# nv-tlabs/GEN3C

Measured on NVIDIA H100. Metric: denoise-steps/sec, 7B DiT, 121-frame 720p latent, higher is better.
Workload: dtype bf16

## Files before the change

### gen3c_b200/csrc/attn_wgmma.cu

```cuda
#include <cmath>
#include <cstdlib>

#include "kernels.h"

namespace g3c {

constexpr int ATT_THREADS = 384;
constexpr int ATT_TILE = 128;
constexpr int ATT_HALF_BYTES = 128 * 128;
constexpr int ATT_TILE_BYTES = 2 * ATT_HALF_BYTES;
constexpr int ATT_STAGES = 2;
constexpr int ATT_SMEM = ATT_TILE_BYTES + ATT_STAGES * 2 * ATT_TILE_BYTES + 256 + 1024;

struct AttnParams {
  int Lq, Lk, heads;
  int ldo;
  int vt_chunk_len;
  __nv_bfloat16* O;
  float scale_log2;
  const uint32_t* chunk_flags;
  uint32_t flag_seq;
  int first_chunk;
  unsigned long long peer_timeout_ns;
  unsigned long long* wait_ns;
  unsigned long long* trace;
};

static unsigned long long* g_attn_trace = nullptr;

#define ATT_TR(role, slot)                                                                                  \
  do {                                                                                                      \
    if constexpr (kTrace) {                                                                                 \
      if (blockIdx.x == 0 && blockIdx.y == 0 && j < 64 && (threadIdx.x % 128) == 0)                         \
        p.trace[((role) * 64 + j) * 8 + (slot)] = clock64();                                                \
    }                                                                                                       \
  } while (0)

__device__ __forceinline__ float ex2_approx(float x) {
  float y;
  asm("ex2.approx.ftz.f32 %0, %1;\n" : "=f"(y) : "f"(x));
  return y;
}

template <bool kTrace>
__global__ void __launch_bounds__(ATT_THREADS, 1)
    k_attn_fwd(const __grid_constant__ CUtensorMap tmQ, const __grid_constant__ CUtensorMap tmK,
               const __grid_constant__ CUtensorMap tmV, const AttnParams p) {
  extern __shared__ uint8_t smem_raw[];
  uint8_t* smem = reinterpret_cast<uint8_t*>((reinterpret_cast<uintptr_t>(smem_raw) + 1023) &
                                             ~static_cast<uintptr_t>(1023));
  uint8_t* smem_q = smem;
  uint8_t* smem_k = smem + ATT_TILE_BYTES;
  uint8_t* smem_v = smem_k + ATT_STAGES * ATT_TILE_BYTES;
  uint64_t* bars = reinterpret_cast<uint64_t*>(smem_v + ATT_STAGES * ATT_TILE_BYTES);
  uint64_t* q_full = bars;
  uint64_t* k_full = bars + 1;
  uint64_t* v_full = bars + 1 + ATT_STAGES;
  uint64_t* kv_empty = bars + 1 + 2 * ATT_STAGES;

  const uint32_t wg = threadIdx.x / 128;
  const uint32_t tid = threadIdx.x % 128;
  const int head = blockIdx.y;
  const int q0 = blockIdx.x * ATT_TILE;
  const int n_kv = p.Lk / ATT_TILE;

  if (threadIdx.x == 0) {
    tma_prefetch_desc(&tmQ);
    tma_prefetch_desc(&tmK);
    tma_prefetch_desc(&tmV);
    mbar_init(q_full, 1);
    for (int i = 0; i < ATT_STAGES; ++i) {
      mbar_init(&k_full[i], 1);
      mbar_init(&v_full[i], 1);
      mbar_init(&kv_empty[i], 2);
    }
    fence_barrier_init();
  }
  __syncthreads();

  if (wg == 0) {
    setmaxnreg_dec<24>();
    if (tid == 0) {
      mbar_expect_tx(q_full, ATT_TILE_BYTES);
      for (int h = 0; h < 2; ++h) tma_load_2d(smem_q + h * ATT_HALF_BYTES, &tmQ, q_full, head * 128 + h * 64, q0);
      const int tiles_per_chunk = p.vt_chunk_len / ATT_TILE;
      const int n_chunks = p.Lk / p.vt_chunk_len;
      uint32_t stage = 0, phase = 0;
      for (int j = 0; j < n_kv; ++j) {
        int chunk = p.first_chunk + j / tiles_per_chunk;
        if (chunk >= n_chunks) chunk -= n_chunks;
        const int within = j % tiles_per_chunk;
        if (p.chunk_flags && within == 0 && chunk != p.first_chunk) {
          uint32_t v, spins = 0;
          uint64_t t0 = 0;
          for (;;) {
            asm volatile("ld.acquire.sys.global.u32 %0, [%1];\n" : "=r"(v) : "l"(p.chunk_flags + chunk) : "memory");
            if ((int)(v - p.flag_seq) >= 0) break;
            if (t0 == 0) t0 = global_timer_ns();
            if ((++spins & 0x3FFu) == 0 && global_timer_ns() - t0 > p.peer_timeout_ns) asm volatile("trap;\n");
          }
          if (t0 != 0 && p.wait_ns) atomicAdd(p.wait_ns, (unsigned long long)(global_timer_ns() - t0));
          asm volatile("fence.proxy.async.global;\n" ::: "memory");
        }
        const int kv0 = chunk * p.vt_chunk_len + within * ATT_TILE;
        mbar_wait_ns(&kv_empty[stage], phase ^ 1, p.peer_timeout_ns);
        mbar_expect_tx(&k_full[stage], ATT_TILE_BYTES);
        for (int h = 0; h < 2; ++h)
          tma_load_2d(smem_k + stage * ATT_TILE_BYTES + h * ATT_HALF_BYTES, &tmK, &k_full[stage], head * 128 + h * 64,
                      kv0);
        mbar_expect_tx(&v_full[stage], ATT_TILE_BYTES);
        for (int h = 0; h < 2; ++h)
          tma_load_3d(smem_v + stage * ATT_TILE_BYTES + h * ATT_HALF_BYTES, &tmV, &v_full[stage],
                      within * ATT_TILE + h * 64, head * 128, chunk);
        if (++stage == ATT_STAGES) {
          stage = 0;
          phase ^= 1;
        }
      }
    }
  } else {
    setmaxnreg_inc<240>();
    const uint32_t c = wg - 1;
    const uint32_t warp = tid / 32, lane = tid % 32;
    float o[64];
#pragma unroll
    for (int i = 0; i < 64; ++i) o[i] = 0.f;
    float m_run[2] = {-INFINITY, -INFINITY};
    float l_run[2] = {0.f, 0.f};
    const float sl2 = p.scale_log2;
    const uint64_t dq = make_sdesc_sw128(smem_u32(smem_q + c * 64 * 128));
    mbar_wait_ns(q_full, 0, p.peer_timeout_ns);
    uint32_t stage = 0, phase = 0;
    for (int j = 0; j < n_kv; ++j) {
      ATT_TR(1 + c, 0);
      float s[64];
      mbar_wait_ns(&k_full[stage], phase, p.peer_timeout_ns);
      ATT_TR(1 + c, 1);
      {
        const uint64_t dk = make_sdesc_sw128(smem_u32(smem_k + stage * ATT_TILE_BYTES));
        wgmma_fence();
#pragma unroll
        for (int kk = 0; kk < 8; ++kk) {
          const uint32_t off = (kk >> 2) * ATT_HALF_BYTES + (kk & 3) * 32;
          wgmma_ss_n128(s, sdesc_advance(dq, off), sdesc_advance(dk, off), kk > 0 ? 1u : 0u);
        }
        wgmma_commit();
        wgmma_wait<0>();
        fence_regs(s);
      }
      ATT_TR(1 + c, 2);
      float mx[2] = {-INFINITY, -INFINITY};
#pragma unroll
      for (int i = 0; i < 16; ++i) {
        mx[0] = fmaxf(mx[0], fmaxf(s[4 * i], s[4 * i + 1]));
        mx[1] = fmaxf(mx[1], fmaxf(s[4 * i + 2], s[4 * i + 3]));
      }
      float alpha[2], nm[2];
#pragma unroll
      for (int h = 0; h < 2; ++h) {
        mx[h] = fmaxf(mx[h], __shfl_xor_sync(0xffffffffu, mx[h], 1));
        mx[h] = fmaxf(mx[h], __shfl_xor_sync(0xffffffffu, mx[h], 2));
        nm[h] = fmaxf(m_run[h], mx[h] * sl2);
        alpha[h] = ex2_approx(m_run[h] - nm[h]);
        m_run[h] = nm[h];
        l_run[h] *= alpha[h];
      }
      uint32_t pa[32];
#pragma unroll
      for (int i = 0; i < 16; ++i) {
        const float p0 = ex2_approx(fmaf(s[4 * i], sl2, -nm[0])), p1 = ex2_approx(fmaf(s[4 * i + 1], sl2, -nm[0]));
        const float p2 = ex2_approx(fmaf(s[4 * i + 2], sl2, -nm[1])), p3 = ex2_approx(fmaf(s[4 * i + 3], sl2, -nm[1]));
        l_run[0] += p0 + p1;
        l_run[1] += p2 + p3;
        pa[2 * i] = pack_bf16x2(p0, p1);
        pa[2 * i + 1] = pack_bf16x2(p2, p3);
      }
#pragma unroll
      for (int i = 0; i < 16; ++i) {
        o[4 * i] *= alpha[0];
        o[4 * i + 1] *= alpha[0];
        o[4 * i + 2] *= alpha[1];
        o[4 * i + 3] *= alpha[1];
      }
      ATT_TR(1 + c, 3);
      mbar_wait_ns(&v_full[stage], phase, p.peer_timeout_ns);
      {
        const uint64_t dv = make_sdesc_sw128(smem_u32(smem_v + stage * ATT_TILE_BYTES));
        wgmma_fence();
#pragma unroll
        for (int kk = 0; kk < 8; ++kk) {
          const uint32_t a[4] = {pa[4 * kk], pa[4 * kk + 1], pa[4 * kk + 2], pa[4 * kk + 3]};
          wgmma_rs_n128(o, a, sdesc_advance(dv, (kk >> 2) * ATT_HALF_BYTES + (kk & 3) * 32));
        }
        wgmma_commit();
        wgmma_wait<0>();
        fence_regs(o);
      }
      if (tid == 0) mbar_arrive(&kv_empty[stage]);
      ATT_TR(1 + c, 4);
      if (++stage == ATT_STAGES) {
        stage = 0;
        phase ^= 1;
      }
    }
    float inv[2];
#pragma unroll
    for (int h = 0; h < 2; ++h) {
      float l = l_run[h];
      l += __shfl_xor_sync(0xffffffffu, l, 1);
      l += __shfl_xor_sync(0xffffffffu, l, 2);
      inv[h] = 1.0f / l;
    }
    const int row_a = q0 + (int)(c * 64 + warp * 16 + lane / 4);
#pragma unroll
    for (int h = 0; h < 2; ++h) {
      const int row = row_a + 8 * h;
      if (row >= p.Lq) continue;
      __nv_bfloat16* dst = p.O + (size_t)row * p.ldo + head * 128 + 2 * (lane % 4);
#pragma unroll
      for (int i = 0; i < 16; ++i)
        *reinterpret_cast<uint32_t*>(dst + 8 * i) = pack_bf16x2(o[4 * i + 2 * h] * inv[h], o[4 * i + 2 * h + 1] * inv[h]);
    }
  }
}

int attn_fwd(const void* q, const void* k, const void* vt, void* o, int Lq, int Lk, int heads,
             int ldq, int ldk, int ldo, int vt_chunk_len, float scale, cudaStream_t st, const ChunkGate* gate) {
  G3C_REQUIRE(q && k && vt && o, "attn: null operand");
  G3C_REQUIRE(Lq > 0 && Lk > 0 && heads > 0, "attn: bad sizes");
  G3C_REQUIRE(Lk % ATT_TILE == 0, "attn: Lk=%d must be a multiple of 128", Lk);
  if (vt_chunk_len <= 0) vt_chunk_len = Lk;
  G3C_REQUIRE(Lk % vt_chunk_len == 0 && vt_chunk_len % ATT_TILE == 0,
              "attn: vt_chunk_len=%d must divide Lk=%d and be a multiple of 128", vt_chunk_len, Lk);
  G3C_REQUIRE(ldq % 8 == 0 && ldk % 8 == 0 && ldo % 8 == 0 && ldq >= heads * 128 &&
                  ldk >= heads * 128 && ldo >= heads * 128,
              "attn: leading dimensions must be >= heads*128 and multiples of 8");
  G3C_REQUIRE((reinterpret_cast<uintptr_t>(o) & 15) == 0, "attn: O must be 16-byte aligned");
  CUtensorMap tmQ, tmK, tmV;
  {
    uint64_t dims[2] = {(uint64_t)heads * 128, (uint64_t)Lq}, str[1] = {(uint64_t)ldq * 2};
    uint32_t box[2] = {64, 128};
    int rc = make_tmap_bf16_sw128(&tmQ, q, 2, dims, str, box);
    if (rc) return rc;
  }
  {
    uint64_t dims[2] = {(uint64_t)heads * 128, (uint64_t)Lk}, str[1] = {(uint64_t)ldk * 2};
    uint32_t box[2] = {64, 128};
    int rc = make_tmap_bf16_sw128(&tmK, k, 2, dims, str, box);
    if (rc) return rc;
  }
  {
    const int chunks = Lk / vt_chunk_len;
    uint64_t dims[3] = {(uint64_t)vt_chunk_len, (uint64_t)heads * 128, (uint64_t)chunks};
    uint64_t str[2] = {(uint64_t)vt_chunk_len * 2, (uint64_t)vt_chunk_len * 2 * heads * 128};
    uint32_t box[3] = {64, 128, 1};
    int rc = make_tmap_bf16_sw128(&tmV, vt, 3, dims, str, box);
    if (rc) return rc;
  }
  static bool configured = false;
  if (!configured) {
    G3C_CUDA(cudaFuncSetAttribute(k_attn_fwd<false>, cudaFuncAttributeMaxDynamicSharedMemorySize, ATT_SMEM));
    G3C_CUDA(cudaFuncSetAttribute(k_attn_fwd<true>, cudaFuncAttributeMaxDynamicSharedMemorySize, ATT_SMEM));
    configured = true;
  }
  AttnParams p;
  p.Lq = Lq;
  p.Lk = Lk;
  p.heads = heads;
  p.ldo = ldo;
  p.vt_chunk_len = vt_chunk_len;
  p.O = reinterpret_cast<__nv_bfloat16*>(o);
  p.scale_log2 = scale * 1.4426950408889634f;
  if (fabsf(p.scale_log2 - 1.0f) < 1e-6f) p.scale_log2 = 1.0f;
  p.chunk_flags = gate ? gate->flags : nullptr;
  p.peer_timeout_ns = gate ? peer_timeout_ns() : G3C_MBAR_TIMEOUT_NS;
  p.wait_ns = gate ? gate->wait_ns : nullptr;
  p.flag_seq = gate ? gate->seq : 0;
  p.first_chunk = gate ? gate->first : 0;
  p.trace = g_attn_trace;
  G3C_REQUIRE(p.first_chunk >= 0 && p.first_chunk < Lk / vt_chunk_len, "attn: first chunk %d out of range", p.first_chunk);
  dim3 grid((Lq + ATT_TILE - 1) / ATT_TILE, heads);
  if (g_attn_trace) k_attn_fwd<true><<<grid, ATT_THREADS, ATT_SMEM, st>>>(tmQ, tmK, tmV, p);
  else k_attn_fwd<false><<<grid, ATT_THREADS, ATT_SMEM, st>>>(tmQ, tmK, tmV, p);
  G3C_CUDA(cudaGetLastError());
  return G3C_OK;
}

}

extern "C" int g3c_attn_set_trace(unsigned long long* device_buffer) {
  g3c::g_attn_trace = device_buffer;
  return G3C_OK;
}

extern "C" int g3c_attn_fwd(const void* q, const void* k, const void* vt, void* o, int Lq, int Lk,
                            int heads, int ldq, int ldk, int ldo, int vt_chunk_len, float scale,
                            void* stream) {
  return g3c::attn_fwd(q, k, vt, o, Lq, Lk, heads, ldq, ldk, ldo, vt_chunk_len, scale,
                       (cudaStream_t)stream, nullptr);
}
```

### gen3c_b200/csrc/common.cuh

```cuda
#pragma once
#include <cuda.h>
#include <cuda_bf16.h>
#include <cuda_runtime.h>
#include <stdint.h>
#include <stdio.h>

#include "../../include/gen3c_b200.h"
#include "wgmma_ops.cuh"

namespace g3c {

void set_error(const char* fmt, ...);
int cuda_fail(cudaError_t e, const char* what, const char* file, int line);
#define G3C_CUDA(x)                                                         \
  do {                                                                      \
    cudaError_t _e = (x);                                                   \
    if (_e != cudaSuccess) return ::g3c::cuda_fail(_e, #x, __FILE__, __LINE__); \
  } while (0)
#define G3C_REQUIRE(cond, ...)        \
  do {                                \
    if (!(cond)) {                    \
      ::g3c::set_error(__VA_ARGS__);  \
      return G3C_EINVAL;       \
    }                                 \
  } while (0)

int make_tmap_bf16_sw128(CUtensorMap* out, const void* base, int rank, const uint64_t* dims,
                         const uint64_t* strides_bytes, const uint32_t* box);
int make_tmap_f32_sw128(CUtensorMap* out, const void* base, const uint64_t* dims,
                        const uint64_t* strides_bytes, const uint32_t* box);

int sm_count();

#ifdef __CUDACC__
__device__ __forceinline__ uint32_t smem_u32(const void* p) {
  return static_cast<uint32_t>(__cvta_generic_to_shared(p));
}
__device__ __forceinline__ uint32_t lane_id() { return threadIdx.x & 31; }
__device__ __forceinline__ uint32_t warp_id() { return __shfl_sync(0xffffffffu, threadIdx.x >> 5, 0); }

__device__ __forceinline__ bool elect_one() {
  uint32_t pred = 0;
  asm volatile(
      "{\n\t.reg .pred P;\n\t"
      "elect.sync _|P, 0xffffffff;\n\t"
      "selp.b32 %0, 1, 0, P;\n\t}\n"
      : "=r"(pred));
  return pred != 0;
}

__device__ __forceinline__ void mbar_init(uint64_t* bar, uint32_t count) {
  asm volatile("mbarrier.init.shared::cta.b64 [%0], %1;\n" ::"r"(smem_u32(bar)), "r"(count));
}
__device__ __forceinline__ void fence_barrier_init() {
  asm volatile("fence.mbarrier_init.release.cluster;\n" ::: "memory");
}
__device__ __forceinline__ void fence_proxy_async() {
  asm volatile("fence.proxy.async.shared::cta;\n" ::: "memory");
}
__device__ __forceinline__ void mbar_expect_tx(uint64_t* bar, uint32_t bytes) {
  asm volatile("mbarrier.arrive.expect_tx.shared::cta.b64 _, [%0], %1;\n" ::"r"(smem_u32(bar)),
               "r"(bytes)
               : "memory");
}
__device__ __forceinline__ void mbar_arrive(uint64_t* bar) {
  asm volatile("mbarrier.arrive.shared::cta.b64 _, [%0];\n" ::"r"(smem_u32(bar)) : "memory");
}
#ifndef G3C_MBAR_SUSPEND_NS
#define G3C_MBAR_SUSPEND_NS 0
#endif
__device__ __forceinline__ bool mbar_try_wait(uint64_t* bar, uint32_t parity) {
  uint32_t ok;
#if G3C_MBAR_SUSPEND_NS > 0
  asm volatile(
      "{\n\t.reg .pred P;\n\t"
      "mbarrier.try_wait.parity.shared::cta.b64 P, [%1], %2, %3;\n\t"
      "selp.b32 %0, 1, 0, P;\n\t}\n"
      : "=r"(ok)
      : "r"(smem_u32(bar)), "r"(parity), "r"((uint32_t)G3C_MBAR_SUSPEND_NS)
      : "memory");
#else
  asm volatile(
      "{\n\t.reg .pred P;\n\t"
      "mbarrier.try_wait.parity.shared::cta.b64 P, [%1], %2;\n\t"
      "selp.b32 %0, 1, 0, P;\n\t}\n"
      : "=r"(ok)
      : "r"(smem_u32(bar)), "r"(parity)
      : "memory");
#endif
  return ok != 0;
}
__device__ __forceinline__ bool mbar_test(uint64_t* bar, uint32_t parity) {
  uint32_t ok;
  asm volatile(
      "{\n\t.reg .pred P;\n\t"
      "mbarrier.test_wait.parity.shared::cta.b64 P, [%1], %2;\n\t"
      "selp.b32 %0, 1, 0, P;\n\t}\n"
      : "=r"(ok)
      : "r"(smem_u32(bar)), "r"(parity)
      : "memory");
  return ok != 0;
}
#ifndef G3C_MBAR_TIMEOUT_NS
#define G3C_MBAR_TIMEOUT_NS 4000000000ull
#endif
__device__ __forceinline__ uint64_t global_timer_ns() {
  uint64_t t;
  asm volatile("mov.u64 %0, %%globaltimer;\n" : "=l"(t));
  return t;
}
#ifdef G3C_MBAR_DEBUG
#define G3C_MBAR_TIMEOUT_ACTION(bar, parity)                                                                 \
  do {                                                                                                       \
    printf("g3c: mbarrier timeout block(%d,%d) thread %d bar@%u parity %u\n", blockIdx.x, blockIdx.y,        \
           threadIdx.x, bar, parity);                                                                        \
    __trap();                                                                                                \
  } while (0)
#else
#define G3C_MBAR_TIMEOUT_ACTION(bar, parity) asm volatile("trap;\n")
#endif
__device__ __forceinline__ void mbar_wait(uint64_t* bar, uint32_t parity) {
  if (mbar_try_wait(bar, parity)) return;
  uint32_t spins = 0;
  uint64_t t0 = 0;
  while (!mbar_try_wait(bar, parity)) {
    if ((++spins & 0xFFFu) == 0) {
      uint64_t now = global_timer_ns();
      if (t0 == 0) t0 = now;
      else if (now - t0 > G3C_MBAR_TIMEOUT_NS) G3C_MBAR_TIMEOUT_ACTION(smem_u32(bar), parity);
    }
  }
}

__device__ __forceinline__ void mbar_wait_ns(uint64_t* bar, uint32_t parity, unsigned long long timeout_ns) {
  if (mbar_try_wait(bar, parity)) return;
  uint32_t spins = 0;
  uint64_t t0 = 0;
  while (!mbar_try_wait(bar, parity)) {
    if ((++spins & 0xFFFu) == 0) {
      uint64_t now = global_timer_ns();
      if (t0 == 0) t0 = now;
      else if (now - t0 > timeout_ns) G3C_MBAR_TIMEOUT_ACTION(smem_u32(bar), parity);
    }
  }
}

__device__ __forceinline__ void tma_prefetch_desc(const CUtensorMap* m) {
  asm volatile("prefetch.tensormap [%0];\n" ::"l"(reinterpret_cast<uint64_t>(m)) : "memory");
}
__device__ __forceinline__ void tma_load_2d(void* smem_dst, const CUtensorMap* m, uint64_t* bar,
                                            int c0, int c1) {
  asm volatile(
      "cp.async.bulk.tensor.2d.shared::cluster.global.mbarrier::complete_tx::bytes"
      " [%0], [%1, {%3, %4}], [%2];\n" ::"r"(smem_u32(smem_dst)),
      "l"(reinterpret_cast<uint64_t>(m)), "r"(smem_u32(bar)), "r"(c0), "r"(c1)
      : "memory");
}
__device__ __forceinline__ void tma_load_3d(void* smem_dst, const CUtensorMap* m, uint64_t* bar,
                                            int c0, int c1, int c2) {
  asm volatile(
      "cp.async.bulk.tensor.3d.shared::cluster.global.mbarrier::complete_tx::bytes"
      " [%0], [%1, {%3, %4, %5}], [%2];\n" ::"r"(smem_u32(smem_dst)),
      "l"(reinterpret_cast<uint64_t>(m)), "r"(smem_u32(bar)), "r"(c0), "r"(c1), "r"(c2)
      : "memory");
}

__device__ __forceinline__ void tma_store_2d(const CUtensorMap* m, const void* smem_src, int c0, int c1) {
  asm volatile("cp.async.bulk.tensor.2d.global.shared::cta.bulk_group [%0, {%2, %3}], [%1];\n" ::"l"(
                   reinterpret_cast<uint64_t>(m)),
               "r"(smem_u32(smem_src)), "r"(c0), "r"(c1)
               : "memory");
}
__device__ __forceinline__ void tma_reduce_add_2d(const CUtensorMap* m, const void* smem_src, int c0, int c1) {
  asm volatile("cp.reduce.async.bulk.tensor.2d.global.shared::cta.add.bulk_group [%0, {%2, %3}], [%1];\n" ::"l"(
                   reinterpret_cast<uint64_t>(m)),
               "r"(smem_u32(smem_src)), "r"(c0), "r"(c1)
               : "memory");
}
__device__ __forceinline__ void tma_store_commit() { asm volatile("cp.async.bulk.commit_group;\n" ::: "memory"); }
template <int N>
__device__ __forceinline__ void tma_store_wait_read() {
  asm volatile("cp.async.bulk.wait_group.read %0;\n" ::"n"(N) : "memory");
}
template <int N>
__device__ __forceinline__ void tma_store_wait_all() {
  asm volatile("cp.async.bulk.wait_group %0;\n" ::"n"(N) : "memory");
}

__device__ __forceinline__ void wgmma_fence() { asm volatile("wgmma.fence.sync.aligned;\n" ::: "memory"); }
__device__ __forceinline__ void wgmma_commit() { asm volatile("wgmma.commit_group.sync.aligned;\n" ::: "memory"); }
template <int N>
__device__ __forceinline__ void wgmma_wait() {
  asm volatile("wgmma.wait_group.sync.aligned %0;\n" ::"n"(N) : "memory");
}
template <int N>
__device__ __forceinline__ void fence_regs(float (&r)[N]) {
#pragma unroll
  for (int i = 0; i < N; ++i) asm volatile("" : "+f"(r[i])::"memory");
}

__device__ __forceinline__ uint64_t make_sdesc_sw128(uint32_t smem_addr) {
  uint64_t d = 0;
  d |= static_cast<uint64_t>((smem_addr & 0x3FFFFu) >> 4);
  d |= static_cast<uint64_t>(1) << 16;
  d |= static_cast<uint64_t>(1024u >> 4) << 32;
  d |= static_cast<uint64_t>(1) << 62;
  return d;
}
__device__ __forceinline__ uint64_t sdesc_advance(uint64_t d, uint32_t bytes) {
  return d + static_cast<uint64_t>(bytes >> 4);
}

template <int N>
__device__ __forceinline__ void setmaxnreg_dec() {
  asm volatile("setmaxnreg.dec.sync.aligned.u32 %0;\n" ::"n"(N));
}
template <int N>
__device__ __forceinline__ void setmaxnreg_inc() {
  asm volatile("setmaxnreg.inc.sync.aligned.u32 %0;\n" ::"n"(N));
}

__device__ __forceinline__ uint32_t pack_bf16x2(float lo, float hi) {
  __nv_bfloat162 v = __floats2bfloat162_rn(lo, hi);
  return *reinterpret_cast<uint32_t*>(&v);
}
__device__ __forceinline__ float warp_max(float v) {
#pragma unroll
  for (int o = 16; o > 0; o >>= 1) v = fmaxf(v, __shfl_xor_sync(0xffffffffu, v, o));
  return v;
}
__device__ __forceinline__ float warp_sum(float v) {
#pragma unroll
  for (int o = 16; o > 0; o >>= 1) v += __shfl_xor_sync(0xffffffffu, v, o);
  return v;
}
#endif

}
```

### gen3c_b200/csrc/dit_engine.cu

```cuda
#include <dlfcn.h>

#include <array>
#include <cmath>
#include <cstdlib>
#include <cstring>
#include <string>
#include <unordered_map>
#include <vector>

#include "kernels.h"

namespace g3c {

typedef struct ncclComm* ncclComm_t;
typedef struct { char internal[128]; } ncclUniqueId;
struct NcclApi {
  int (*GetUniqueId)(ncclUniqueId*) = nullptr;
  int (*CommInitRank)(ncclComm_t*, int, ncclUniqueId, int) = nullptr;
  int (*CommDestroy)(ncclComm_t) = nullptr;
  int (*AllGather)(const void*, void*, size_t, int, ncclComm_t, cudaStream_t) = nullptr;
  int (*GroupStart)() = nullptr;
  int (*GroupEnd)() = nullptr;
  const char* (*GetErrorString)(int) = nullptr;
  bool ok = false;
// ... 242 lines not shown
  if (!v) {
    const char* e = getenv("G3C_PEER_TIMEOUT_S");
    double sec = e ? atof(e) : 600.0;
    if (!(sec > 0)) sec = 600.0;
    v = (unsigned long long)(sec * 1e9);
  }
  return v;
}

static int build_tables(g3c_dit* h, cudaStream_t st) {
  if (h->tables_ready) return G3C_OK;
  const g3c_dit_config& c = h->cfg;
  const int dim = 128, dim_h = dim / 6 * 2, dim_w = dim_h, dim_t = dim - 2 * dim_h;
  const int nt = dim_t / 2, nh = dim_h / 2, nw = dim_w / 2;
  std::vector<float> fr(64);
  auto ntk = [](float ratio, int d) { return powf(ratio, (float)d / (float)(d - 2)); };
  const float th_h = 10000.0f * ntk(c.rope_h_ratio, dim_h), th_w = 10000.0f * ntk(c.rope_w_ratio, dim_w),
              th_t = 10000.0f * ntk(c.rope_t_ratio, dim_t);
  for (int j = 0; j < nt; ++j) fr[j] = 1.0f / powf(th_t, (float)(2 * j) / (float)dim_t);
  for (int j = 0; j < nh; ++j) fr[nt + j] = 1.0f / powf(th_h, (float)(2 * j) / (float)dim_h);
  for (int j = 0; j < nw; ++j) fr[nt + nh + j] = 1.0f / powf(th_w, (float)(2 * j) / (float)dim_w);
  G3C_CUDA(cudaMemcpyAsync(h->freqs, fr.data(), 64 * sizeof(float), cudaMemcpyHostToDevice, st));
  G3C_CUDA(cudaStreamSynchronize(st));
  const int t0 = h->cp_rank * h->T;
  const float t_scale = (1.0f / h->fps) * (float)c.base_fps;
  TRY(rope_table(h->freqs, nt, nh, nw, t0, t_scale, h->T, h->Hp, h->Wp, h->rope, st));
  TRY(abs_pos(h->pos_t, h->pos_h, h->pos_w, t0, h->T, h->Hp, h->Wp, c.model_channels, h->pos, st));
  h->tables_ready = true;
  return G3C_OK;
}

static int forward(g3c_dit* h, const void* x_in, const void* cond_mask, const void* cond_pose,
                   const void* padding_mask, float timestep, const void* ctx, void* out,
                   cudaStream_t st) {
  static_assert(sizeof(float) == 4, "");
  G3C_REQUIRE(h && x_in && cond_mask && ctx && out, "dit_forward: null argument");
  G3C_REQUIRE(h->L > 0, "dit_forward: g3c_dit_set_shape was not called");
  TRY(resolve(h, st));
  TRY(build_tables(h, st));
  const g3c_dit_config& c = h->cfg;
  const int D = c.model_channels, R = c.adaln_lora_dim, F = c.ffn_dim, L = h->L, heads = c.num_heads;
  const int Lk_all = L * h->cp_size;
  const float attn_scale = 0.6931471805599453f;
  static int fuse_nr = -1;
  if (fuse_nr < 0) {
    const char* e = getenv("G3C_FUSE_NORM_ROPE");
    fuse_nr = e ? atoi(e) != 0 : 1;
  }
  auto proj_norm_rope = [&](const void* a, const void* w, __nv_bfloat16* out, int M, int Kin,
                            const float* gamma, const float* cs, int& launches) -> int {
    if (fuse_nr) {
      NormRope nr;
      nr.gamma = gamma;
      nr.cs = cs;
      nr.eps = 1e-6f;
      TRY(prof_mark(h, CAT_GEMM, true, st));
      TRY(gemm_bf16(a, w, out, M, D, Kin, Kin, Kin, D, G3C_EPI_BF16, nullptr, 0, st, nullptr, &nr));
      TRY(prof_mark(h, CAT_GEMM, false, st));
      launches += 1;
    } else {
      TRY(prof_mark(h, CAT_GEMM, true, st));
      TRY(gemm_bf16(a, w, out, M, D, Kin, Kin, Kin, D, G3C_EPI_BF16, nullptr, 0, st));
      TRY(prof_mark(h, CAT_GEMM, false, st));
      TRY(prof_mark(h, CAT_ELTWISE, true, st));
      TRY(rmsnorm_rope(out, D, M, heads, gamma, cs, 1e-6f, st));
      TRY(prof_mark(h, CAT_ELTWISE, false, st));
      launches += 2;
    }
    return G3C_OK;
  };
  int n = 0;

  PatchSrc src;
  src.ptr[0] = (const __nv_bfloat16*)x_in;        src.nch[0] = 16;                      src.per_frame[0] = 1;
  src.ptr[1] = (const __nv_bfloat16*)cond_mask;   src.nch[1] = 1;                       src.per_frame[1] = 1;
  src.ptr[2] = (const __nv_bfloat16*)cond_pose;   src.nch[2] = c.in_channels - 17;      src.per_frame[2] = 1;
  src.ptr[3] = (const __nv_bfloat16*)padding_mask; src.nch[3] = c.concat_padding_mask ? 1 : 0; src.per_frame[3] = 0;
  K(CAT_ELTWISE, patchify(src, h->T, h->Hp, h->Wp, h->Kpad, h->tok, st));
  K(CAT_GEMM, gemm_bf16(h->tok, h->w_patch_pad, h->x, L, D, h->Kpad, h->Kpad, h->Kpad, D, G3C_EPI_F32, nullptr, 0, st));

  if (!(h->mods_valid && h->mods_timestep == timestep)) {
    K(CAT_VECTOR, timestep_embed(timestep, D, h->affine_gamma, 1e-6f, h->vec_s, h->vec_emb, st));
    K(CAT_VECTOR, gemv(h->w_t1, h->vec_s, nullptr, h->vec_h1, D, D, 0, 0, st));
    K(CAT_VECTOR, gemv(h->w_t2, h->vec_h1, nullptr, h->vec_lora, 3 * D, D, 1, 0, st));
    for (int i = 0; i < c.num_blocks; ++i)
      for (int j = 0; j < 3; ++j) {
        const SubBlock& s = h->blk[i][j];
        K(CAT_VECTOR, gemv(s.ada1, h->vec_emb, nullptr, h->vec_a, R, D, 1, 0, st));
        K(CAT_VECTOR, gemv(s.ada2, h->vec_a, h->vec_lora, h->mods + (size_t)(i * 3 + j) * 3 * D, 3 * D, R, 0, 0, st));
      }
    K(CAT_VECTOR, gemv(h->f_ada1, h->vec_emb, nullptr, h->vec_a, R, D, 1, 0, st));
    K(CAT_VECTOR, gemv(h->f_ada2, h->vec_a, h->vec_lora, h->modf, 2 * D, R, 0, 0, st));
    h->mods_valid = true;
    h->mods_timestep = timestep;
  }

  __nv_bfloat16* k_loc = h->k_all + (size_t)h->cp_rank * L * D;
  __nv_bfloat16* vt_loc = h->vt_all + (size_t)h->cp_rank * L * D;

  for (int i = 0; i < c.num_blocks; ++i) {
    {
      const SubBlock& s = h->blk[i][0];
      const float* m = h->mods + (size_t)(i * 3 + 0) * 3 * D;
      K(CAT_ELTWISE, ln_modulate(h->x, h->pos, m, m + D, h->xn, L, D, 1e-6f, st));
      if (h->cp_size > 1 && h->cp_p2p) {
        G3C_REQUIRE(h->peers_open, "dit_forward: context-parallel peers not imported (g3c_dit_cp_import)");
        const uint32_t seq = ++h->kv_seq;
        const int set = seq & 1, me = h->cp_rank;
        const size_t slice = (size_t)L * D * 2;
        char* reg = (char*)h->cp_region;
        __nv_bfloat16* kb = (__nv_bfloat16*)(reg + h->off_k[set]);
        __nv_bfloat16* vb = (__nv_bfloat16*)(reg + h->off_vt[set]);
        __nv_bfloat16* kl = kb + (size_t)me * L * D;
        __nv_bfloat16* vl = vb + (size_t)me * L * D;
        PeerDst pk, pv, pf;
        for (int r = 0; r < h->cp_size; ++r) {
          char* pb = (char*)h->peer_base[r];
          pf.ptr[pf.n++] = pb + h->off_flags + (size_t)(set * 8 + me) * 4;
          if (r == me) continue;
          pk.ptr[pk.n++] = pb + h->off_k[set] + (size_t)me * slice;
          pv.ptr[pv.n++] = pb + h->off_vt[set] + (size_t)me * slice;
        }
        if (h->cp_push_sm) {
          K(CAT_GEMM, gemm_bf16(h->xn, s.wk, kl, L, D, D, D, D, D, G3C_EPI_BF16, nullptr, 0, st));
          K(CAT_COMM, rmsnorm_rope(kl, D, L, heads, s.gk, h->rope, 1e-6f, st, &pk));
          K(CAT_COMM, gemm_bf16(s.wv, h->xn, vl, D, L, D, D, D, L, G3C_EPI_BF16, nullptr, 0, st, &pv));
          k_cp_signal<<<1, 32, 0, st>>>(pf, seq);
          G3C_CUDA(cudaGetLastError());
          ++n;
        } else {
          TRY(proj_norm_rope(h->xn, s.wk, kl, L, D, s.gk, h->rope, n));
          K(CAT_GEMM, gemm_bf16(s.wv, h->xn, vl, D, L, D, D, D, L, G3C_EPI_BF16, nullptr, 0, st));
          G3C_CUDA(cudaEventRecord(h->ev_kv, st));
          G3C_CUDA(cudaStreamWaitEvent(h->comm_stream, h->ev_kv, 0));
          uint32_t* slot = h->seq_ring + (seq % g3c_dit::kSeqRing);
          *slot = seq;
          for (int i2 = 1; i2 < h->cp_size; ++i2) {
            const int r = (me - i2 + h->cp_size) % h->cp_size;
            char* pb = (char*)h->peer_base[r];
            G3C_CUDA(cudaMemcpyAsync(pb + h->off_k[set] + (size_t)me * slice, kl, slice, cudaMemcpyDeviceToDevice,
                                     h->comm_stream));
            G3C_CUDA(cudaMemcpyAsync(pb + h->off_vt[set] + (size_t)me * slice, vl, slice, cudaMemcpyDeviceToDevice,
                                     h->comm_stream));
            G3C_CUDA(cudaMemcpyAsync(pb + h->off_flags + (size_t)(set * 8 + me) * 4, slot, 4, cudaMemcpyHostToDevice,
                                     h->comm_stream));
          }
        }
        TRY(proj_norm_rope(h->xn, s.wq, h->q, L, D, s.gq, h->rope, n));
        ChunkGate gate;
        gate.flags = (const uint32_t*)(reg + h->off_flags) + set * 8;
        gate.seq = seq;
        gate.first = me;
        gate.wait_ns = h->prof ? h->wait_ns : nullptr;
        h->wait_cta_launches = (double)((L + 255) / 256) * heads;
        K(CAT_ATTN_SELF, attn_fwd(h->q, kb, vb, h->att, L, Lk_all, heads, D, D, D, L, attn_scale, st, &gate));
      } else {
        TRY(proj_norm_rope(h->xn, s.wk, k_loc, L, D, s.gk, h->rope, n));
        K(CAT_GEMM, gemm_bf16(s.wv, h->xn, vt_loc, D, L, D, D, D, L, G3C_EPI_BF16, nullptr, 0, st));
        if (h->cp_size > 1) {
          G3C_CUDA(cudaEventRecord(h->ev_kv, st));
          G3C_CUDA(cudaStreamWaitEvent(h->comm_stream, h->ev_kv, 0));
          G3C_NCCL(nccl().GroupStart());
          G3C_NCCL(nccl().AllGather(k_loc, h->k_all, (size_t)L * D, kNcclBfloat16, h->comm, h->comm_stream));
          G3C_NCCL(nccl().AllGather(vt_loc, h->vt_all, (size_t)L * D, kNcclBfloat16, h->comm, h->comm_stream));
          G3C_NCCL(nccl().GroupEnd());
          G3C_CUDA(cudaEventRecord(h->ev_gathered, h->comm_stream));
          n += 2;
        }
        TRY(proj_norm_rope(h->xn, s.wq, h->q, L, D, s.gq, h->rope, n));
        if (h->cp_size > 1) G3C_CUDA(cudaStreamWaitEvent(st, h->ev_gathered, 0));
        K(CAT_ATTN_SELF, attn_fwd(h->q, h->k_all, h->vt_all, h->att, L, Lk_all, heads, D, D, D, L, attn_scale, st));
      }
      K(CAT_GEMM, gemm_bf16(h->att, s.wo, h->x, L, D, D, D, D, D, G3C_EPI_GATED_RESIDUAL_F32, m + 2 * D, 0, st));
    }
    {
      const SubBlock& s = h->blk[i][1];
      const float* m = h->mods + (size_t)(i * 3 + 1) * 3 * D;
      const int C = c.context_dim, M = h->ctx_len;
      K(CAT_ELTWISE, ln_modulate(h->x, nullptr, m, m + D, h->xn, L, D, 1e-6f, st));
      TRY(proj_norm_rope(ctx, s.wk, h->kc, M, C, s.gk, nullptr, n));
      K(CAT_GEMM, gemm_bf16(s.wv, ctx, h->vtc, D, M, C, C, C, M, G3C_EPI_BF16, nullptr, 0, st));
      TRY(proj_norm_rope(h->xn, s.wq, h->q, L, D, s.gq, nullptr, n));
      K(CAT_ATTN_CROSS, attn_fwd(h->q, h->kc, h->vtc, h->att, L, M, heads, D, D, D, M, attn_scale, st));
      K(CAT_GEMM, gemm_bf16(h->att, s.wo, h->x, L, D, D, D, D, D, G3C_EPI_GATED_RESIDUAL_F32, m + 2 * D, 0, st));
    }
    {
      const SubBlock& s = h->blk[i][2];
      const float* m = h->mods + (size_t)(i * 3 + 2) * 3 * D;
      K(CAT_ELTWISE, ln_modulate(h->x, nullptr, m, m + D, h->xn, L, D, 1e-6f, st));
      K(CAT_GEMM, gemm_bf16(h->xn, s.w1, h->hid, L, F, D, D, D, F, G3C_EPI_GELU_BF16, nullptr, 0, st));
      K(CAT_GEMM, gemm_bf16(h->hid, s.w2, h->x, L, D, F, F, F, D, G3C_EPI_GATED_RESIDUAL_F32, m + 2 * D, 0, st));
    }
  }
  const int No = c.out_channels * 4;
  K(CAT_ELTWISE, ln_modulate(h->x, nullptr, h->modf, h->modf + D, h->xn, L, D, 1e-6f, st));
  K(CAT_GEMM, gemm_bf16(h->xn, h->w_final, h->yfin, L, No, D, D, D, No, G3C_EPI_F32, nullptr, 64, st));
  K(CAT_ELTWISE, unpatchify(h->yfin, No, h->T, h->Hp, h->Wp, c.out_channels, (__nv_bfloat16*)out, st));
  h->launches = n;
  return G3C_OK;
}

}

extern "C" {

int g3c_dit_create(const g3c_dit_config* cfg, g3c_dit_t** out) {
  G3C_REQUIRE(cfg && out, "dit_create: null argument");
  G3C_REQUIRE(cfg->model_channels % 128 == 0 && cfg->num_heads * 128 == cfg->model_channels,
              "dit_create: head_dim must be 128 (model_channels=%d heads=%d)", cfg->model_channels,
              cfg->num_heads);
  G3C_REQUIRE(cfg->adaln_lora_dim % 8 == 0 && cfg->context_dim % 8 == 0 && cfg->ffn_dim % 8 == 0,
              "dit_create: adaln_lora_dim/context_dim/ffn_dim must be multiples of 8");
  G3C_REQUIRE(cfg->in_channels >= 17 && cfg->out_channels > 0 && cfg->num_blocks > 0, "dit_create: bad config");
  g3c_dit* h = new g3c_dit();
  h->cfg = *cfg;
  *out = h;
  return G3C_OK;
}

static void free_cp_region(g3c_dit* h) {
  if (h->cp_region || h->cfg_region) cudaDeviceSynchronize();
  if (h->cfg_peer) cudaIpcCloseMemHandle(h->cfg_peer);
  h->cfg_peer = nullptr;
  if (h->cfg_region) cudaFree(h->cfg_region);
  h->cfg_region = nullptr;
  for (int r = 0; r < 8; ++r) {
    if (h->peer_base[r] && h->peer_base[r] != h->cp_region) cudaIpcCloseMemHandle(h->peer_base[r]);
    h->peer_base[r] = nullptr;
  }
  h->peers_open = false;
  if (h->cp_region) cudaFree(h->cp_region);
  h->cp_region = nullptr;
  h->cp_region_bytes = 0;
}

static void free_ws(g3c_dit* h) {
  free_cp_region(h);
  if (h->ws) cudaFree(h->ws);
  h->ws = nullptr;
  h->ws_bytes = 0;
  h->L = 0;
  h->tables_ready = false;
  h->mods_valid = false;
}

int g3c_dit_destroy(g3c_dit_t* h) {
  if (!h) return G3C_OK;
  free_ws(h);
  if (h->w_patch_pad) cudaFree(h->w_patch_pad);
  if (h->gammas) cudaFree(h->gammas);
  if (h->comm && nccl().ok) nccl().CommDestroy(h->comm);
  if (h->comm_stream) cudaStreamDestroy(h->comm_stream);
  if (h->seq_ring) cudaFreeHost(h->seq_ring);
  if (h->wait_ns) cudaFree(h->wait_ns);
  if (h->ev_kv) cudaEventDestroy(h->ev_kv);
  if (h->ev_gathered) cudaEventDestroy(h->ev_gathered);
  for (cudaEvent_t e : h->ev_pool) cudaEventDestroy(e);
  delete h;
  return G3C_OK;
}

int g3c_dit_load(g3c_dit_t* h, const char* name, const void* ptr, const int64_t* shape, int ndim, int dtype) {
  G3C_REQUIRE(h && name && ptr && shape && ndim >= 1 && ndim <= 4, "dit_load: bad arguments");
  WTensor t;
  t.ptr = ptr;
  t.shape.assign(shape, shape + ndim);
  t.dtype = dtype;
  h->w[name] = t;
  h->resolved = false;
  h->tables_ready = false;
  h->mods_valid = false;
  return G3C_OK;
}

int g3c_nccl_unique_id(void* out128) {
  G3C_REQUIRE(out128, "nccl_unique_id: null argument");
  if (!nccl().ok) {
    set_error("libnccl.so.2 could not be loaded");
    return G3C_ENCCL;
  }
  ncclUniqueId id;
  G3C_NCCL(nccl().GetUniqueId(&id));
  memcpy(out128, &id, 128);
  return G3C_OK;
}

int g3c_dit_enable_cp(g3c_dit_t* h, const void* nccl_unique_id, int cp_rank, int cp_size) {
  G3C_REQUIRE(h && cp_size >= 1 && cp_size <= 8 && cp_rank >= 0 && cp_rank < cp_size, "enable_cp: bad arguments");
  if (h->comm && nccl().ok) {
    nccl().CommDestroy(h->comm);
    h->comm = nullptr;
  }
  h->cp_p2p = nccl_unique_id == nullptr;
  {
    const char* e = getenv("G3C_CP_PUSH");
    h->cp_push_sm = e && e[0] == 's';
  }
  if (!h->cp_p2p) {
    if (!nccl().ok) {
      set_error("libnccl.so.2 could not be loaded");
      return G3C_ENCCL;
    }
    ncclUniqueId id;
    memcpy(&id, nccl_unique_id, 128);
    G3C_NCCL(nccl().CommInitRank(&h->comm, cp_size, id, cp_rank));
  }
  if (!h->comm_stream) {
// ... 278 lines not shown
```

### gen3c_b200/csrc/kernels.h

```cpp
#pragma once
#include "common.cuh"

namespace g3c {

struct PeerDst {
  int n = 0;
  void* ptr[8] = {nullptr, nullptr, nullptr, nullptr, nullptr, nullptr, nullptr, nullptr};
};

struct NormRope {
  const float* gamma = nullptr;
  const float* cs = nullptr;
  float eps = 1e-6f;
};

int gemm_bf16(const void* A, const void* B, void* D, int M, int N, int K, int lda, int ldb, int ldd,
              int epilogue, const float* gate, int block_n, cudaStream_t st, const PeerDst* peers = nullptr,
              const NormRope* norm_rope = nullptr);
struct ChunkGate {
  const uint32_t* flags = nullptr;
  uint32_t seq = 0;
  int first = 0;
  unsigned long long* wait_ns = nullptr;
};
unsigned long long peer_timeout_ns();
int attn_fwd(const void* q, const void* k, const void* vt, void* o, int Lq, int Lk, int heads,
             int ldq, int ldk, int ldo, int vt_chunk_len, float scale, cudaStream_t st,
             const ChunkGate* gate = nullptr);

struct PatchSrc {
  const __nv_bfloat16* ptr[4];
  int nch[4];
  int per_frame[4];
};

int ln_modulate(float* x, const __nv_bfloat16* pos, const float* shift, const float* scale,
                __nv_bfloat16* y, int L, int D, float eps, cudaStream_t st);
int rmsnorm_rope(__nv_bfloat16* qk, int ld, int L, int heads, const float* gamma, const float* cs,
                 float eps, cudaStream_t st, const PeerDst* peers = nullptr);
int gemv(const __nv_bfloat16* W, const float* x, const float* add, float* y, int N, int K, int pre,
         int round_out, cudaStream_t st);
int patchify(const PatchSrc& src, int T, int Hp, int Wp, int Kpad, __nv_bfloat16* out, cudaStream_t st);
int unpatchify(const float* y, int ldy, int T, int Hp, int Wp, int C, __nv_bfloat16* out, cudaStream_t st);
int timestep_embed(float t, int D, const __nv_bfloat16* gamma, float eps, float* s, float* emb,
                   cudaStream_t st);
int abs_pos(const __nv_bfloat16* pt, const __nv_bfloat16* ph, const __nv_bfloat16* pw, int t0, int T,
            int Hp, int Wp, int D, __nv_bfloat16* out, cudaStream_t st);
int rope_table(const float* freqs, int nt, int nh, int nw, int t0, float t_scale, int T, int Hp, int Wp,
               float* cs, cudaStream_t st);
int bf16_to_f32(const __nv_bfloat16* in, float* out, size_t n, cudaStream_t st, float scale = 1.0f);
int sampler_pre(const __nv_bfloat16* xt, const __nv_bfloat16* gt, const float* noise, const float* ind_t,
                int C, int T, size_t plane, float sigma, float sigma_aug, float sd,
                __nv_bfloat16* xtilde, __nv_bfloat16* xin, cudaStream_t st);
int sampler_post(const __nv_bfloat16* xtilde, const __nv_bfloat16* oc, const __nv_bfloat16* ou,
                 const __nv_bfloat16* gt, const float* ind_t, int C, int T, size_t plane, float guidance,
                 float sigma, float sigma_next, float sigma_aug, float sd, __nv_bfloat16* xnext,
                 __nv_bfloat16* net_out, cudaStream_t st);

}
```

Measured before the change: 0.09124.

## Software-pipeline attention: overlap next QK^T with softmax and PV, ping-pong warpgroups

Restructures the consumer loop of the wgmma attention kernel so the QK^T for tile j is issued together with the PV product for tile j-1, letting the softmax run while tensor-core work is in flight. It adds turn barriers that alternate wgmma issue between the two consumer warpgroups, and splits the K and V empty barriers so K slots free earlier. Prologue and epilogue handle the first S and the last PV. It also adds an exit-on-timeout wait and a done barrier for the producer. The cost is more live registers (s, pa and o held at once) and extra barrier traffic.

```diff
diff --git a/gen3c_b200/csrc/attn_wgmma.cu b/gen3c_b200/csrc/attn_wgmma.cu
--- a/gen3c_b200/csrc/attn_wgmma.cu
+++ b/gen3c_b200/csrc/attn_wgmma.cu
@@ -6,11 +6,13 @@
 namespace g3c {
 
 constexpr int ATT_THREADS = 384;
-constexpr int ATT_TILE = 128;
+constexpr int ATT_TILE = ATT_ROWS_PER_CTA;
 constexpr int ATT_HALF_BYTES = 128 * 128;
 constexpr int ATT_TILE_BYTES = 2 * ATT_HALF_BYTES;
 constexpr int ATT_STAGES = 2;
 constexpr int ATT_SMEM = ATT_TILE_BYTES + ATT_STAGES * 2 * ATT_TILE_BYTES + 256 + 1024;
+static_assert(ATT_SMEM <= 227 * 1024, "attention: Q + K/V rings exceed the 227 KB of shared memory per block");
+static_assert(1 + 4 * ATT_STAGES + 3 <= 256 / 8, "attention: barriers exceed their 256-byte area");
 
 struct AttnParams {
   int Lq, Lk, heads;
@@ -42,6 +44,61 @@
   return y;
 }
 
+__device__ __forceinline__ void softmax_tile(float (&s)[64], float (&m_run)[2], float (&l_run)[2], float (&alpha)[2],
+                                             float sl2) {
+  float mx[2] = {-INFINITY, -INFINITY};
+#pragma unroll
+  for (int i = 0; i < 16; ++i) {
+    mx[0] = fmaxf(mx[0], fmaxf(s[4 * i], s[4 * i + 1]));
+    mx[1] = fmaxf(mx[1], fmaxf(s[4 * i + 2], s[4 * i + 3]));
+  }
+  float nm[2];
+#pragma unroll
+  for (int h = 0; h < 2; ++h) {
+    mx[h] = fmaxf(mx[h], __shfl_xor_sync(0xffffffffu, mx[h], 1));
+    mx[h] = fmaxf(mx[h], __shfl_xor_sync(0xffffffffu, mx[h], 2));
+    nm[h] = fmaxf(m_run[h], mx[h] * sl2);
+    alpha[h] = ex2_approx(m_run[h] - nm[h]);
+    m_run[h] = nm[h];
+    l_run[h] *= alpha[h];
+  }
+#pragma unroll
+  for (int i = 0; i < 16; ++i) {
+    s[4 * i] = ex2_approx(fmaf(s[4 * i], sl2, -nm[0]));
+    s[4 * i + 1] = ex2_approx(fmaf(s[4 * i + 1], sl2, -nm[0]));
+    s[4 * i + 2] = ex2_approx(fmaf(s[4 * i + 2], sl2, -nm[1]));
+    s[4 * i + 3] = ex2_approx(fmaf(s[4 * i + 3], sl2, -nm[1]));
+    l_run[0] += s[4 * i] + s[4 * i + 1];
+    l_run[1] += s[4 * i + 2] + s[4 * i + 3];
+  }
+}
+
+__device__ __forceinline__ void issue_s(float (&s)[64], uint64_t dq, const uint8_t* k_tile) {
+  const uint64_t dk = make_sdesc_sw128(smem_u32(k_tile));
+#pragma unroll
+  for (int kk = 0; kk < 8; ++kk) {
+    const uint32_t off = (kk >> 2) * ATT_HALF_BYTES + (kk & 3) * 32;
+    wgmma_ss_n128(s, sdesc_advance(dq, off), sdesc_advance(dk, off), kk > 0 ? 1u : 0u);
+  }
+}
+
+__device__ __forceinline__ void issue_pv(float (&o)[64], const uint32_t (&pa)[32], const uint8_t* v_tile) {
+  const uint64_t dv = make_sdesc_sw128(smem_u32(v_tile));
+#pragma unroll
+  for (int kk = 0; kk < 8; ++kk) {
+    const uint32_t a[4] = {pa[4 * kk], pa[4 * kk + 1], pa[4 * kk + 2], pa[4 * kk + 3]};
+    wgmma_rs_n128(o, a, sdesc_advance(dv, (kk >> 2) * ATT_HALF_BYTES + (kk & 3) * 32));
+  }
+}
+
+__device__ __forceinline__ void pack_p(uint32_t (&pa)[32], const float (&s)[64]) {
+#pragma unroll
+  for (int i = 0; i < 16; ++i) {
+    pa[2 * i] = pack_bf16x2(s[4 * i], s[4 * i + 1]);
+    pa[2 * i + 1] = pack_bf16x2(s[4 * i + 2], s[4 * i + 3]);
+  }
+}
+
 template <bool kTrace>
 __global__ void __launch_bounds__(ATT_THREADS, 1)
     k_attn_fwd(const __grid_constant__ CUtensorMap tmQ, const __grid_constant__ CUtensorMap tmK,
@@ -55,8 +112,11 @@
   uint64_t* bars = reinterpret_cast<uint64_t*>(smem_v + ATT_STAGES * ATT_TILE_BYTES);
   uint64_t* q_full = bars;
   uint64_t* k_full = bars + 1;
-  uint64_t* v_full = bars + 1 + ATT_STAGES;
-  uint64_t* kv_empty = bars + 1 + 2 * ATT_STAGES;
+  uint64_t* v_full = k_full + ATT_STAGES;
+  uint64_t* k_empty = v_full + ATT_STAGES;
+  uint64_t* v_empty = k_empty + ATT_STAGES;
+  uint64_t* turn = v_empty + ATT_STAGES;
+  uint64_t* done = turn + 2;
 
   const uint32_t wg = threadIdx.x / 128;
   const uint32_t tid = threadIdx.x % 128;
@@ -72,8 +132,12 @@
     for (int i = 0; i < ATT_STAGES; ++i) {
       mbar_init(&k_full[i], 1);
       mbar_init(&v_full[i], 1);
-      mbar_init(&kv_empty[i], 2);
-    }
+      mbar_init(&k_empty[i], 2);
+      mbar_init(&v_empty[i], 2);
+    }
+    for (int c = 0; c < 2; ++c) mbar_init(&turn[c], 4);
+    for (int w = 0; w < 4; ++w) mbar_arrive(&turn[0]);
+    mbar_init(done, 2);
     fence_barrier_init();
   }
   __syncthreads();
@@ -103,11 +167,12 @@
           asm volatile("fence.proxy.async.global;\n" ::: "memory");
         }
         const int kv0 = chunk * p.vt_chunk_len + within * ATT_TILE;
-        mbar_wait_ns(&kv_empty[stage], phase ^ 1, p.peer_timeout_ns);
+        mbar_wait_ns(&k_empty[stage], phase ^ 1, p.peer_timeout_ns);
         mbar_expect_tx(&k_full[stage], ATT_TILE_BYTES);
         for (int h = 0; h < 2; ++h)
           tma_load_2d(smem_k + stage * ATT_TILE_BYTES + h * ATT_HALF_BYTES, &tmK, &k_full[stage], head * 128 + h * 64,
                       kv0);
+        mbar_wait_ns(&v_empty[stage], phase ^ 1, p.peer_timeout_ns);
         mbar_expect_tx(&v_full[stage], ATT_TILE_BYTES);
         for (int h = 0; h < 2; ++h)
           tma_load_3d(smem_v + stage * ATT_TILE_BYTES + h * ATT_HALF_BYTES, &tmV, &v_full[stage],
@@ -117,64 +182,72 @@
           phase ^= 1;
         }
       }
+      mbar_wait_ns(done, 0, p.peer_timeout_ns);
     }
   } else {
     setmaxnreg_inc<240>();
     const uint32_t c = wg - 1;
     const uint32_t warp = tid / 32, lane = tid % 32;
+    const unsigned long long tmo = p.peer_timeout_ns;
     float o[64];
 #pragma unroll
     for (int i = 0; i < 64; ++i) o[i] = 0.f;
+    float s[64];
+    uint32_t pa[32];
     float m_run[2] = {-INFINITY, -INFINITY};
     float l_run[2] = {0.f, 0.f};
+    float alpha[2];
     const float sl2 = p.scale_log2;
     const uint64_t dq = make_sdesc_sw128(smem_u32(smem_q + c * 64 * 128));
-    mbar_wait_ns(q_full, 0, p.peer_timeout_ns);
-    uint32_t stage = 0, phase = 0;
-    for (int j = 0; j < n_kv; ++j) {
+    uint32_t tph = 0;
+    uint32_t ks = 0, kp = 0;
+    uint32_t vs = 0, vp = 0;
+    int j = 0;
+    mbar_wait_ns_or_exit(q_full, 0, tmo);
+    mbar_wait_ns_or_exit(&k_full[ks], kp, tmo);
+    mbar_wait_ns_or_exit(&turn[c], tph, tmo);
+    tph ^= 1;
+    ATT_TR(1 + c, 0);
+    wgmma_fence();
+    issue_s(s, dq, smem_k + ks * ATT_TILE_BYTES);
+    wgmma_commit();
+    if (lane == 0) mbar_arrive(&turn[c ^ 1]);
+    ATT_TR(1 + c, 1);
+    wgmma_wait<0>();
+    fence_regs(s);
+    if (tid == 0) mbar_arrive(&k_empty[ks]);
+    ATT_TR(1 + c, 2);
+    softmax_tile(s, m_run, l_run, alpha, sl2);
+    pack_p(pa, s);
+    ATT_TR(1 + c, 3);
+    if (++ks == ATT_STAGES) {
+      ks = 0;
+      kp ^= 1;
+    }
+    for (j = 1; j < n_kv; ++j) {
+      mbar_wait_ns_or_exit(&k_full[ks], kp, tmo);
+      mbar_wait_ns_or_exit(&v_full[vs], vp, tmo);
+      mbar_wait_ns_or_exit(&turn[c], tph, tmo);
+      tph ^= 1;
       ATT_TR(1 + c, 0);
-      float s[64];
-      mbar_wait_ns(&k_full[stage], phase, p.peer_timeout_ns);
+      wgmma_fence();
+      issue_s(s, dq, smem_k + ks * ATT_TILE_BYTES);
+      wgmma_commit();
+      issue_pv(o, pa, smem_v + vs * ATT_TILE_BYTES);
+      wgmma_commit();
+      if (lane == 0) mbar_arrive(&turn[c ^ 1]);
       ATT_TR(1 + c, 1);
-      {
-        const uint64_t dk = make_sdesc_sw128(smem_u32(smem_k + stage * ATT_TILE_BYTES));
-        wgmma_fence();
-#pragma unroll
-        for (int kk = 0; kk < 8; ++kk) {
-          const uint32_t off = (kk >> 2) * ATT_HALF_BYTES + (kk & 3) * 32;
-          wgmma_ss_n128(s, sdesc_advance(dq, off), sdesc_advance(dk, off), kk > 0 ? 1u : 0u);
-        }
-        wgmma_commit();
-        wgmma_wait<0>();
-        fence_regs(s);
-      }
+      wgmma_wait<1>();
+      fence_regs(s);
+      if (tid == 0) mbar_arrive(&k_empty[ks]);
       ATT_TR(1 + c, 2);
-      float mx[2] = {-INFINITY, -INFINITY};
-#pragma unroll
-      for (int i = 0; i < 16; ++i) {
-        mx[0] = fmaxf(mx[0], fmaxf(s[4 * i], s[4 * i + 1]));
-        mx[1] = fmaxf(mx[1], fmaxf(s[4 * i + 2], s[4 * i + 3]));
-      }
-      float alpha[2], nm[2];
-#pragma unroll
-      for (int h = 0; h < 2; ++h) {
-        mx[h] = fmaxf(mx[h], __shfl_xor_sync(0xffffffffu, mx[h], 1));
-        mx[h] = fmaxf(mx[h], __shfl_xor_sync(0xffffffffu, mx[h], 2));
-        nm[h] = fmaxf(m_run[h], mx[h] * sl2);
-        alpha[h] = ex2_approx(m_run[h] - nm[h]);
-        m_run[h] = nm[h];
-        l_run[h] *= alpha[h];
-      }
-      uint32_t pa[32];
-#pragma unroll
-      for (int i = 0; i < 16; ++i) {
-        const float p0 = ex2_approx(fmaf(s[4 * i], sl2, -nm[0])), p1 = ex2_approx(fmaf(s[4 * i + 1], sl2, -nm[0]));
-        const float p2 = ex2_approx(fmaf(s[4 * i + 2], sl2, -nm[1])), p3 = ex2_approx(fmaf(s[4 * i + 3], sl2, -nm[1]));
-        l_run[0] += p0 + p1;
-        l_run[1] += p2 + p3;
-        pa[2 * i] = pack_bf16x2(p0, p1);
-        pa[2 * i + 1] = pack_bf16x2(p2, p3);
-      }
+      softmax_tile(s, m_run, l_run, alpha, sl2);
+      ATT_TR(1 + c, 3);
+      wgmma_wait<0>();
+      fence_regs(o);
+      fence_regs(pa);
+      if (tid == 0) mbar_arrive(&v_empty[vs]);
+      ATT_TR(1 + c, 4);
 #pragma unroll
       for (int i = 0; i < 16; ++i) {
         o[4 * i] *= alpha[0];
@@ -182,27 +255,29 @@
         o[4 * i + 2] *= alpha[1];
         o[4 * i + 3] *= alpha[1];
       }
-      ATT_TR(1 + c, 3);
-      mbar_wait_ns(&v_full[stage], phase, p.peer_timeout_ns);
-      {
-        const uint64_t dv = make_sdesc_sw128(smem_u32(smem_v + stage * ATT_TILE_BYTES));
-        wgmma_fence();
-#pragma unroll
-        for (int kk = 0; kk < 8; ++kk) {
-          const uint32_t a[4] = {pa[4 * kk], pa[4 * kk + 1], pa[4 * kk + 2], pa[4 * kk + 3]};
-          wgmma_rs_n128(o, a, sdesc_advance(dv, (kk >> 2) * ATT_HALF_BYTES + (kk & 3) * 32));
-        }
-        wgmma_commit();
-        wgmma_wait<0>();
-        fence_regs(o);
+      pack_p(pa, s);
+      if (++ks == ATT_STAGES) {
+        ks = 0;
+        kp ^= 1;
       }
-      if (tid == 0) mbar_arrive(&kv_empty[stage]);
-      ATT_TR(1 + c, 4);
-      if (++stage == ATT_STAGES) {
-        stage = 0;
-        phase ^= 1;
+      if (++vs == ATT_STAGES) {
+        vs = 0;
+        vp ^= 1;
       }
     }
+    mbar_wait_ns_or_exit(&v_full[vs], vp, tmo);
+    mbar_wait_ns_or_exit(&turn[c], tph, tmo);
+    ATT_TR(1 + c, 0);
+    wgmma_fence();
+    issue_pv(o, pa, smem_v + vs * ATT_TILE_BYTES);
+    wgmma_commit();
+    if (lane == 0) mbar_arrive(&turn[c ^ 1]);
+    ATT_TR(1 + c, 1);
+    wgmma_wait<0>();
+    fence_regs(o);
+    fence_regs(pa);
+    if (tid == 0) mbar_arrive(&v_empty[vs]);
+    ATT_TR(1 + c, 4);
     float inv[2];
 #pragma unroll
     for (int h = 0; h < 2; ++h) {
@@ -221,6 +296,7 @@
       for (int i = 0; i < 16; ++i)
         *reinterpret_cast<uint32_t*>(dst + 8 * i) = pack_bf16x2(o[4 * i + 2 * h] * inv[h], o[4 * i + 2 * h + 1] * inv[h]);
     }
+    if (tid == 0) mbar_arrive(done);
   }
 }
 
diff --git a/gen3c_b200/csrc/common.cuh b/gen3c_b200/csrc/common.cuh
--- a/gen3c_b200/csrc/common.cuh
+++ b/gen3c_b200/csrc/common.cuh
@@ -145,6 +145,19 @@
   }
 }
 
+__device__ __forceinline__ void mbar_wait_ns_or_exit(uint64_t* bar, uint32_t parity, unsigned long long timeout_ns) {
+  if (mbar_try_wait(bar, parity)) return;
+  uint32_t spins = 0;
+  uint64_t t0 = 0;
+  while (!mbar_try_wait(bar, parity)) {
+    if ((++spins & 0xFFFu) == 0) {
+      uint64_t now = global_timer_ns();
+      if (t0 == 0) t0 = now;
+      else if (now - t0 > timeout_ns) asm volatile("exit;\n");
+    }
+  }
+}
+
 __device__ __forceinline__ void tma_prefetch_desc(const CUtensorMap* m) {
   asm volatile("prefetch.tensormap [%0];\n" ::"l"(reinterpret_cast<uint64_t>(m)) : "memory");
 }
@@ -197,6 +210,11 @@
 __device__ __forceinline__ void fence_regs(float (&r)[N]) {
 #pragma unroll
   for (int i = 0; i < N; ++i) asm volatile("" : "+f"(r[i])::"memory");
+}
+template <int N>
+__device__ __forceinline__ void fence_regs(uint32_t (&r)[N]) {
+#pragma unroll
+  for (int i = 0; i < N; ++i) asm volatile("" : "+r"(r[i])::"memory");
 }
 
 __device__ __forceinline__ uint64_t make_sdesc_sw128(uint32_t smem_addr) {
diff --git a/gen3c_b200/csrc/dit_engine.cu b/gen3c_b200/csrc/dit_engine.cu
--- a/gen3c_b200/csrc/dit_engine.cu
+++ b/gen3c_b200/csrc/dit_engine.cu
@@ -418,7 +418,7 @@
         gate.seq = seq;
         gate.first = me;
         gate.wait_ns = h->prof ? h->wait_ns : nullptr;
-        h->wait_cta_launches = (double)((L + 255) / 256) * heads;
+        h->wait_cta_launches = (double)((L + ATT_ROWS_PER_CTA - 1) / ATT_ROWS_PER_CTA) * heads;
         K(CAT_ATTN_SELF, attn_fwd(h->q, kb, vb, h->att, L, Lk_all, heads, D, D, D, L, attn_scale, st, &gate));
       } else {
         TRY(proj_norm_rope(h->xn, s.wk, k_loc, L, D, s.gk, h->rope, n));
diff --git a/gen3c_b200/csrc/kernels.h b/gen3c_b200/csrc/kernels.h
--- a/gen3c_b200/csrc/kernels.h
+++ b/gen3c_b200/csrc/kernels.h
@@ -24,6 +24,7 @@
   unsigned long long* wait_ns = nullptr;
 };
 unsigned long long peer_timeout_ns();
+constexpr int ATT_ROWS_PER_CTA = 128;
 int attn_fwd(const void* q, const void* k, const void* vt, void* o, int Lq, int Lk, int heads,
              int ldq, int ldk, int ldo, int vt_chunk_len, float scale, cudaStream_t st,
              const ChunkGate* gate = nullptr);
```

After: 0.09470, median of 6. 3.8% higher.
